# michaelklachko/NoisyNet

Hardware: NVIDIA H100
Metric: NoisyNet CIFAR-10 4-bit training images/sec (higher is better)
Workload: dtype bf16

## Files before the change

include/noisynet_b200.h:

```cpp
#ifndef NOISYNET_B200_H
#define NOISYNET_B200_H

#include <stdint.h>

#ifdef __cplusplus
extern "C" {
#endif

#define NN_ABI_VERSION 16


typedef struct nn_rng {
    uint64_t seed;
    uint64_t offset;
    const uint64_t* offset_dev;
} nn_rng;

const char* nn_last_error(void);
int nn_abi_version(void);
uint64_t nn_launch_count(void);
int nn_device_info(int device, int* sm_count, int* cc_major, int* cc_minor);
int nn_rng_advance(uint64_t* offset_dev, uint64_t inc, int device, void* stream);


int nn_quantize_fwd(const float* x, float* y, int64_t n, int bits, double min_value,
                    double max_value, float stochastic, const float* u_inject, nn_rng rng,
                    int device, void* stream);
int nn_quantize_bwd(const float* x, const float* gy, float* gx, int64_t n, double min_value,
                    double max_value, int device, void* stream);

int64_t nn_range_scratch_bytes(void);
int nn_range_select(const float* x, int64_t n, int64_t k_rank, double pctl_percent, int mode, double min_value, float* out4,
// ... 63 lines not shown
    int64_t workspace_bytes;
    const void* x_packed;
    const void* w_packed;
    int32_t w_packed_layout;
    float* pooled_out;
    uint8_t* argmax_out;
    float* bn_mean;
    float* bn_invstd;
    float* bn_running_mean;
    float* bn_running_var;
    float bn_eps, bn_momentum;
    int32_t bn_eval_mode;
    void* bn_scratch;
    float* zero_out;
} nn_conv_fwd_args;
int64_t nn_conv_bn_scratch_bytes(int Cout);
int nn_conv_linear_bn_fusable(const nn_conv_geom* g, int32_t noise_mode, int32_t precision, int device);

#define NN_PACK_TILED 0
#define NN_PACK_SHIFT 1
#define NN_PACK_TMA 2
int nn_conv_pack_layout(const nn_conv_geom* g, int32_t noise_mode, int32_t precision);
int nn_conv_dgrad_pack_layout(const nn_conv_geom* g, int32_t precision);
int nn_debug_tma_enable(int enable);
int nn_conv_pool_fusable(const nn_conv_geom* g, int32_t noise_mode, int32_t precision);
int nn_debug_shift_enable(int enable);

int64_t nn_conv_workspace_bytes(const nn_conv_geom* g, int32_t precision);
int nn_conv_supported(const nn_conv_geom* g, int32_t precision, int32_t which);
int nn_debug_error_flag(int device, int reset);
float nn_debug_main_kernel_ms(int enable);
int nn_debug_cta_timeline(long long* host_out, int max_ctas);
int nn_noisy_conv_fwd(const nn_conv_fwd_args* a, int device, void* stream);

typedef struct nn_conv_dgrad_args {
    nn_conv_geom g;
    const float* gy;
    const float* w_eff;
    float* gx;
    const float* x_pre; double x_lo, x_hi;
    int32_t precision;
    float w_code_scale;
    void* workspace; int64_t workspace_bytes;
    const void* gy_packed;
    const void* w_packed;
    int32_t w_packed_layout;
// ... 126 lines not shown
```

noisynet_b200/_lib.py:

```python
import ctypes as C
import os

_HERE = os.path.dirname(os.path.abspath(__file__))
LIB_PATH = os.environ.get("NN_LIB_PATH") or os.path.join(_HERE, "lib", "libnoisynet_b200.so")
ABI_VERSION = 16

NOISE_NONE, NOISE_MERGED, NOISE_EXTERNAL = 0, 1, 2
PREC_FP32, PREC_TF32, PREC_BF16 = 0, 1, 2
PACK_TILED, PACK_SHIFT, PACK_TMA = 0, 1, 2

c_f32p = C.c_void_p


class Rng(C.Structure):
    _fields_ = [("seed", C.c_uint64), ("offset", C.c_uint64), ("offset_dev", C.c_void_p)]


class ConvGeom(C.Structure):
    _fields_ = [("B", C.c_int32), ("Cin", C.c_int32), ("H", C.c_int32), ("W", C.c_int32),
                ("Cout", C.c_int32), ("KH", C.c_int32), ("KW", C.c_int32),
                ("stride", C.c_int32), ("pad", C.c_int32)]


class ConvFwdArgs(C.Structure):
    _fields_ = [("g", ConvGeom),
                ("x", C.c_void_p), ("w_eff", C.c_void_p), ("w_raw", C.c_void_p), ("bias", C.c_void_p),
                ("y", C.c_void_p), ("y_noisy", C.c_void_p),
                ("noise_mode", C.c_int32), ("current", C.c_float),
                ("scale_dev", C.c_void_p), ("z_inject", C.c_void_p), ("z_export", C.c_void_p),
                ("sigma_export", C.c_void_p),
                ("rng", Rng),
                ("stats", C.c_void_p),
# ... 109 lines not shown
                                  C.c_void_p, C.c_float, C.c_float, C.c_void_p, C.c_void_p, C.c_void_p, C.c_void_p,
                                  C.c_int, C.c_void_p, C.c_void_p, C.c_int, C.c_void_p]),
    "nn_allreduce_ctl_bytes": (C.c_int64, []),
    "nn_allreduce_start": (C.c_int, [C.POINTER(C.c_void_p), C.c_void_p, C.c_int, C.c_int, C.c_int, C.c_int64, C.c_int64, C.c_int,
                                     C.c_int, C.c_void_p]),
    "nn_allreduce_wait": (C.c_int, [C.c_void_p, C.c_int, C.c_int, C.c_int, C.c_void_p]),
    "nn_head_eval": (C.c_int, [C.c_void_p, C.c_int, C.c_int, C.c_void_p, C.c_void_p, C.c_void_p, C.c_void_p, C.c_float, C.c_void_p,
                               C.c_int, C.c_void_p]),
    "nn_tensor_stats": (C.c_int, [C.c_void_p, C.c_int64, C.c_void_p, C.c_int, C.c_void_p]),
    "nn_clamp_absmax": (C.c_int, [C.c_void_p, C.c_int64, C.c_float, C.c_void_p, C.c_int, C.c_void_p]),
    "nn_noise_epilogue": (C.c_int, [C.c_void_p, C.c_void_p, C.c_void_p, C.c_int64, C.c_int64, C.c_void_p,
                                    C.c_float, C.c_void_p, C.c_void_p, C.c_void_p, Rng, C.c_int, C.c_void_p]),
    "nn_alt_noise": (C.c_int, [C.c_void_p, C.c_void_p, C.c_int64, C.c_int, C.c_float, C.c_void_p,
                               C.c_void_p, Rng, C.c_int, C.c_void_p]),
    "nn_conv_workspace_bytes": (C.c_int64, [C.POINTER(ConvGeom), C.c_int32]),
    "nn_conv_supported": (C.c_int, [C.POINTER(ConvGeom), C.c_int32, C.c_int32]),
    "nn_debug_error_flag": (C.c_int, [C.c_int, C.c_int]),
    "nn_debug_main_kernel_ms": (C.c_float, [C.c_int]),
    "nn_debug_cta_timeline": (C.c_int, [C.c_void_p, C.c_int]),
    "nn_conv_pack_layout": (C.c_int, [C.POINTER(ConvGeom), C.c_int32, C.c_int32]),
    "nn_debug_shift_enable": (C.c_int, [C.c_int]),
    "nn_debug_tma_enable": (C.c_int, [C.c_int]),
    "nn_conv_dgrad_pack_layout": (C.c_int, [C.POINTER(ConvGeom), C.c_int32]),
    "nn_conv_pool_fusable": (C.c_int, [C.POINTER(ConvGeom), C.c_int32, C.c_int32]),
    "nn_classifier_tail": (C.c_int, [C.POINTER(TailArgs), C.c_int, C.c_void_p]),
    "nn_conv_wgrad_pack_layout": (C.c_int, [C.POINTER(ConvGeom), C.c_int32, C.c_int]),
    "nn_conv_gy_planes_bytes": (C.c_int64, [C.POINTER(ConvGeom)]),
    "nn_noisy_conv_fwd": (C.c_int, [C.POINTER(ConvFwdArgs), C.c_int, C.c_void_p]),
    "nn_noisy_conv_dgrad": (C.c_int, [C.POINTER(ConvDgradArgs), C.c_int, C.c_void_p]),
    "nn_conv_wgrad_workspace_bytes": (C.c_int64, [C.POINTER(ConvGeom), C.c_int32, C.c_int]),
    "nn_noisy_conv_wgrad": (C.c_int, [C.POINTER(ConvWgradArgs), C.c_int, C.c_void_p]),
}

_lib = None


class NoisyNetLibraryError(RuntimeError):
    pass


def load():
    global _lib
    if _lib is not None:
        return _lib
    if not os.path.isfile(LIB_PATH):
        raise NoisyNetLibraryError(
# ... 19 lines not shown
```

noisynet_b200/csrc/nn_conv_tma.cu:

```cuda
#include "nn_conv_tma.h"

#include <cuda.h>

#include "nn_wgmma.cuh"

namespace {

constexpr int TC_MAX_STAGES = 8;

struct TmaConvP {
    CUtensorMap map64, map_tail;
    CUtensorMap mapb64, mapb_tail;
    int M, OH, OW, Cout, stride, pad, KW, taps;
    int n_c64, tail_w, nc, gpt, n_groups;
    int n_mma, n_half, n_tiles;
    int stages, a_stage, b_stage, n_prod, tap_bytes;
    float y_scale, s_scale;
    float *y, *y_noisy;
    float current;
    const float* scale_dev;
    const float* z_inject;
    nn_rng rng;
    int* err_flag;
};
// ... 621 lines not shown
    p.taps = w.taps;
    p.partial_tail = reinterpret_cast<float*>(reinterpret_cast<uint8_t*>(c.partial) + w.main_bytes);
    p.OH = c.OH; p.OW = c.OW; p.stride = c.stride; p.pad = c.pad; p.KW = c.KW; p.n_c64 = w.n_c64; p.n_atoms = w.n_atoms;
    p.Mpix = c.B * c.OH * c.OW; p.Cout = c.Cout; p.num_kb = w.num_kb; p.kb_per_split = w.kb_per_split; p.stages = w.stages;
    p.cols_pad = w.cols_pad; p.partial = c.partial; p.err_flag = c.err_flag;
    typedef void (*WgradKernel)(const WgTmaP);
    const int tw = w.tail_w ? (w.taps * 8 + 15) & ~15 : 0;
    const WgradKernel tail = tw == 16 ? k_wgrad_tma<true, 16> : tw == 32 ? k_wgrad_tma<true, 32> : tw == 80 ? k_wgrad_tma<true, 80>
                           : tw == 128 ? k_wgrad_tma<true, 128> : tw == 208 ? k_wgrad_tma<true, 208> : nullptr;
    if (w.tail_w && !tail) return nn_fail("nn_conv_tma: no remainder weight-gradient kernel for%s %lld taps", "", (long long)w.taps);
    NN_ONCE_PER_DEVICE({
        NN_CUDA_OK(cudaFuncSetAttribute(k_wgrad_tma<false, 0>, cudaFuncAttributeMaxDynamicSharedMemorySize, 227 * 1024));
        for (WgradKernel k : {k_wgrad_tma<true, 16>, k_wgrad_tma<true, 32>, k_wgrad_tma<true, 80>, k_wgrad_tma<true, 128>, k_wgrad_tma<true, 208>})
            NN_CUDA_OK(cudaFuncSetAttribute(k, cudaFuncAttributeMaxDynamicSharedMemorySize, 227 * 1024));
    });
    k_wgrad_tma<false, 0><<<dim3(w.tiles_k, w.m_tiles_n, w.splits), WT_THREADS, w.smem_bytes, st>>>(p);
    NN_LAUNCH_OK();
    if (w.tail_w) {
        tail<<<dim3(1, w.m_tiles_n, w.splits), WT_THREADS, w.smem_bytes, st>>>(p);
        NN_LAUNCH_OK();
    }
    return 0;
}
```

noisynet_b200/csrc/nn_conv_tma.h:

```cpp
#pragma once
#include "nn_common.cuh"

struct TmaPlan {
    int Cp, taps, n_c64, tail_w, wt, nc, gpt, n_groups;
    int n_t, n_tiles, n_mma, n_half, main_col, sig_col;
    int stages, a_stage, b_stage, n_prod, threads;
    int tap_bytes;
    size_t smem_bytes, wp_bytes;
};

bool nn_tma_make_plan(int Cin_k, int KH, int KW, int stride, int pad, int n_out, bool has_sigma, int OH, int OW, TmaPlan* out);

struct TmaConvCall {
    TmaPlan pl;
    int B, H, W;
    int OH, OW, KH, KW, stride, pad;
    int Cout;
    const void* xp;
    const void* wp;
    float y_scale, s_scale;
    float* y;
    float* y_noisy;
    int noise_mode;
    float current;
// ... 1 lines not shown
    const float* z_inject;
    nn_rng rng;
    int* err_flag;
    void *ev0, *ev1;
};
int nn_tma_conv_launch(const TmaConvCall& c, int device, cudaStream_t st);

struct TmaWgradPlan {
    int Cp, Coutp, taps, n_c64, tail_w;
    int n_atoms, tiles_k, cols_pad, m_tiles_n, num_kb, kb_per_split, splits, stages;
    size_t smem_bytes, main_bytes, partial_bytes;
};
bool nn_tma_wgrad_plan(int Cin, int KH, int KW, int stride, int pad, int Cout, int64_t Mpix, int device, TmaWgradPlan* out);
struct TmaWgradCall {
    TmaWgradPlan pl;
    int B, H, W, OH, OW, KH, KW, stride, pad, Cout;
    const void* xp;
    const void* gyp;
    float* partial;
    int* err_flag;
};
int nn_tma_wgrad_launch(const TmaWgradCall& c, int device, cudaStream_t st);

int nn_tma_encode_rows(void* map_out, const void* ptr, uint64_t rows, uint64_t cols, uint64_t pitch_bytes);
```

noisynet_b200/csrc/nn_conv_umma.cu:

```cuda
#include <cuda_bf16.h>
#include <stdio.h>
#include <stdlib.h>

#include "nn_common.cuh"
#include "nn_wgmma.cuh"
#include "nn_conv_tma.h"

namespace {

constexpr int UM_BLOCK_M = 128;
constexpr int UM_BLOCK_K = 64;
constexpr int UM_THREADS = 384;
constexpr int UM_ACC_CH = 4;
constexpr int UM_A_STAGE = UM_BLOCK_M * 128;
constexpr int UM_MAX_NT = 120;

struct UmmaP {
    int B, H, W, Cp;
    int KH, KW, stride, pad, OH, OW;
    int M, Cout, n_t, n_mma, num_kb, stages, acc_cols;
    int main_col, sig_col, wsum_col;
    int ring_bytes;
    const __nv_bfloat16* xp;
    const __nv_bfloat16* wp;
// ... 892 lines not shown
            if (c < C) {
                f = __ldg(x + ((int64_t)b * C + c) * HW + p);
                if (code_scale > 0.f) f = rintf(__fdiv_rn(f, code_scale));
            }
            v[j] = __float2bfloat16_rn(f);
        }
        *reinterpret_cast<uint4*>(xp + (pixel * Cp + chunk * 8)) = *reinterpret_cast<const uint4*>(v);
    }
}

struct PackWP {
    const float *w_eff, *w_raw;
    __nv_bfloat16* wp;
    int Cout, Cin, KHW, Cp, n_t, n_mma, num_kb, n_tiles;
    int main_col, sig_col, wsum_col, noise_mode, mode;
    int layout;
    float w_code_scale;
    int q_bits;
    float q_hi, q_scale, q_max, q_stoch;
    const float* u_inject;
    nn_rng rng;
    const int8_t* codes;
    int t_nc64, t_tail, t_nc, t_wt, t_nhalf, t_tapbytes;
};

__device__ __forceinline__ float pack_main_value(const PackWP& p, const NnRng& rs, int64_t idx) {
    if (p.codes) return (float)p.codes[idx];
    if (p.q_bits > 0) {
        const float w = __ldg(p.w_raw + idx);
        float u = 0.f;
        if (p.q_stoch > 0.f) {
            if (p.u_inject) u = __ldg(p.u_inject + idx);
            else {
                const uint4 r = nn_philox(rs, (uint64_t)(idx >> 2));
                const uint32_t rr[4] = {r.x, r.y, r.z, r.w};
                u = nn_usym(rr[idx & 3], p.q_stoch);
            }
        }
        float t = __fadd_rn(__fdiv_rn(__fadd_rn(w, p.q_hi), p.q_scale), u);
        t = rintf(fminf(fmaxf(t, 0.f), p.q_max));
        return 2.f * t - p.q_max;
    }
    float f = __ldg(p.w_eff + idx);
    if (p.w_code_scale > 0.f) f = rintf(__fdiv_rn(f, p.w_code_scale));
    return f;
}

__device__ __forceinline__ void pack_w_job(const PackWP& p, int64_t start, int64_t stride) {
    const NnRng rs = nn_rng_load(p.rng);
    const bool shift = p.layout == 1, tma = p.layout == 2;
    const int64_t total = shift ? (int64_t)p.num_kb * p.n_mma
                          : tma ? (int64_t)p.n_tiles * p.n_mma * p.KHW * (p.t_wt >> 3)
                                : (int64_t)p.n_tiles * p.num_kb * p.n_mma * 8;
    for (int64_t i = start; i < total; i += stride) {
        int j, r, kb, tile, kbase;
        int tap_t = 0, c_first_t = 0;
        int64_t off_t = 0;
        if (tma) {
            const int cpt = p.t_wt >> 3;
            tap_t = (int)(i % p.KHW);
            const int qc = (int)((i / p.KHW) % cpt);
            const int R = (int)(i / ((int64_t)p.KHW * cpt));
            tile = R / p.n_mma; r = R - tile * p.n_mma;
            c_first_t = qc * 8;
            int ci = c_first_t >> 6;
            if (ci > p.t_nc64) ci = p.t_nc64;
            const int w = ci < p.t_nc64 ? 64 : p.t_tail;
            j = (c_first_t - 64 * ci) >> 3;
            const int gi = ci >> 1, slot = ci & 1;
            const int wa = (2 * gi < p.t_nc64) ? 64 : p.t_tail;
            const int wb = (2 * gi + 1 < p.t_nc) ? ((2 * gi + 1 < p.t_nc64) ? 64 : p.t_tail) : 0;
            const int rank = r / p.t_nhalf, rr = r - rank * p.t_nhalf;
            const int swz = w == 64 ? (rr & 7) : (w == 32 ? ((rr >> 1) & 3) : ((rr >> 2) & 1));
// ... 881 lines not shown
    if (p.pooled) {
        if (mode == 0) NN_SHIFT_LAUNCH(0, 16, true); else if (mode == 1) NN_SHIFT_LAUNCH(1, 16, true); else NN_SHIFT_LAUNCH(2, 16, true);
    } else {
        if (mode == 0) NN_SHIFT_LAUNCH(0, 16, false); else if (mode == 1) NN_SHIFT_LAUNCH(1, 16, false); else NN_SHIFT_LAUNCH(2, 16, false);
    }
#undef NN_SHIFT_LAUNCH
    if (g_time_main) cudaEventRecord(g_ev1, st);
    NN_LAUNCH_OK();
    return 0;
}

extern "C" int nn_conv_pack_layout(const nn_conv_geom* g, int32_t noise_mode, int32_t precision) {
    if (!g || precision != NN_PREC_BF16) return NN_PACK_TILED;
    if (make_shift_plan(*g, noise_mode != NN_NOISE_NONE, nullptr)) return NN_PACK_SHIFT;
    int OH, OW;
    nn_out_hw(*g, OH, OW);
    return nn_tma_make_plan(g->Cin, g->KH, g->KW, g->stride, g->pad, g->Cout, noise_mode != NN_NOISE_NONE, OH, OW, nullptr) ? NN_PACK_TMA
                                                                                                                          : NN_PACK_TILED;
}
extern "C" int nn_conv_dgrad_pack_layout(const nn_conv_geom* g, int32_t precision) {
    if (!g || precision != NN_PREC_BF16 || g->stride != 1) return NN_PACK_TILED;
    return nn_tma_make_plan(g->Cout, g->KH, g->KW, 1, g->KH - 1 - g->pad, g->Cin, false, g->H, g->W, nullptr) ? NN_PACK_TMA : NN_PACK_TILED;
}
extern "C" int nn_conv_pool_fusable(const nn_conv_geom* g, int32_t noise_mode, int32_t precision) {
    if (!g || precision != NN_PREC_BF16) return 0;
    if (!make_shift_plan(*g, noise_mode != NN_NOISE_NONE, nullptr)) return 0;
    int OH, OW;
    nn_out_hw(*g, OH, OW);
    const int ngrp = (g->Cout + 3) / 4;
    return g->W % 8 == 0 && g->H % 16 == 0 && OH % 2 == 0 && OW % 2 == 0 && ngrp / 4 <= SH_POOL_IT - 1 && ngrp % 4 <= 1;
}
extern "C" int nn_conv_linear_bn_fusable(const nn_conv_geom* g, int32_t noise_mode, int32_t precision, int device) {
    if (!g || precision != NN_PREC_BF16) return 0;
    int OH, OW;
    nn_out_hw(*g, OH, OW);
    const int M = g->B * OH * OW;
    if (OH * OW != 1 || M % 256 || M > 4096) return 0;
    const Plan pl = make_plan(g->Cin, g->KH * g->KW, g->Cout, true, noise_mode != NN_NOISE_NONE, false, (int64_t)g->B * g->H * g->W, (M + 127) / 128);
    const int ctas = ((M + UM_BLOCK_M - 1) / UM_BLOCK_M) * pl.n_tiles;
    return ctas * 2 <= nn_num_sms(device) && pl.num_kb >= 8 && pl.num_kb / 2 >= 4;
}
extern "C" int64_t nn_conv_bn_scratch_bytes(int Cout) { return 16 + (int64_t)256 * Cout * 2 * sizeof(double); }
extern "C" int nn_debug_shift_enable(int enable) {
    const int prev = g_shift_enable;
    if (enable >= 0) g_shift_enable = enable;
    return prev;
// ... 172 lines not shown
    return make_plan(jb.Cout, jb.KHW, jb.Cin, true, false, false, 0, (jb.m_rows + 127) / 128);
}

static void shift_plan_for_job(const nn_wprep_job& jb, ShiftPlan* sp) {
    const bool noisy = jb.noise_mode != NN_NOISE_NONE;
    sp->n_t = pad_to(jb.Cout, 8); sp->main_col = 0; sp->sig_col = noisy ? sp->n_t : -1;
    sp->n_mma = pad_to(noisy ? 2 * sp->n_t : sp->n_t, 16);
    sp->n_pairs = (jb.KHW + 1) / 2; sp->n_chunks = 2 * sp->n_pairs;
    sp->b_bytes = sp->n_chunks * sp->n_mma * 16; sp->wp_bytes = (size_t)sp->b_bytes;
}

static bool tma_plan_for_job(const nn_wprep_job& jb, TmaPlan* tp) {
    int k = 1;
    while (k * k < jb.KHW) ++k;
    if (k * k != jb.KHW) return false;
    if (jb.mode == 0) return nn_tma_make_plan(jb.Cin, k, k, 1, 0, jb.Cout, jb.noise_mode != NN_NOISE_NONE, 2, 2, tp);
    return nn_tma_make_plan(jb.Cout, k, k, 1, 0, jb.Cin, false, 2, 2, tp);
}

extern "C" int64_t nn_weight_pack_bytes(const nn_wprep_job* jb) {
    if (!jb) return 0;
    if (jb->layout == NN_PACK_TMA) { TmaPlan tp; return tma_plan_for_job(*jb, &tp) ? (int64_t)align_up(tp.wp_bytes, 1024) : 0; }
    if (jb->layout == NN_PACK_SHIFT) { ShiftPlan sp; shift_plan_for_job(*jb, &sp); return (int64_t)align_up(sp.wp_bytes, 1024); }
    return (int64_t)align_up(plan_for_job(*jb).wp_bytes, 1024);
}

extern "C" int nn_prepare_weights(const nn_wprep_job* jobs, int count, int device, void* stream) {
    if (count <= 0) return 0;
    if (count > UM_MAX_PACK_JOBS) return nn_fail("nn_prepare_weights: too many jobs%s (%lld)", "", count);
    NN_SET_DEVICE(device);
    PackJobs pj;
    memset(&pj, 0, sizeof(pj));
    int64_t max_total = 0;
    for (int i = 0; i < count; ++i) {
        const nn_wprep_job& jb = jobs[i];
        if (!jb.w_raw || !jb.packed_out) return nn_fail("nn_prepare_weights: null pointer%s", "");
        if (jb.q_bits > 0 && !(jb.q_hi > 0)) return nn_fail("nn_prepare_weights: symmetric range needs q_hi > 0%s", "");
        Plan pl = plan_for_job(jb);
        TmaPlan tp;
        if (jb.layout == NN_PACK_TMA) {
            if (jb.want_wsum || !tma_plan_for_job(jb, &tp))
                return nn_fail("nn_prepare_weights: NN_PACK_TMA is not served for this job%s (see nn_conv_pack_layout)", "");
        } else if (jb.layout == NN_PACK_SHIFT) {
            if (jb.mode != 0 || jb.Cin > 8 || jb.want_wsum)
                return nn_fail("nn_prepare_weights: NN_PACK_SHIFT needs a forward job with Cin <= 8 and no colsum row%s", "");
            ShiftPlan sp;
            shift_plan_for_job(jb, &sp);
            pl.Cp = 8; pl.n_t = sp.n_t; pl.n_mma = sp.n_mma; pl.num_kb = sp.n_chunks; pl.n_tiles = 1;
            pl.main_col = sp.main_col; pl.sig_col = sp.sig_col; pl.wsum_col = -1;
        }
        PackWP& pw = pj.j[i];
        pw.w_eff = jb.w_raw; pw.w_raw = jb.w_raw; pw.wp = (__nv_bfloat16*)jb.packed_out;
        pw.Cout = jb.Cout; pw.Cin = jb.Cin; pw.KHW = jb.KHW; pw.Cp = pl.Cp; pw.n_t = pl.n_t; pw.n_mma = pl.n_mma;
        pw.num_kb = pl.num_kb; pw.n_tiles = pl.n_tiles; pw.main_col = pl.main_col; pw.sig_col = pl.sig_col;
        pw.wsum_col = pl.wsum_col; pw.noise_mode = jb.noise_mode; pw.mode = jb.mode; pw.w_code_scale = 0.f;
        pw.layout = jb.layout;
        pw.q_bits = jb.q_bits;
        if (jb.q_bits > 0) {
            const double qmax = (double)((1u << jb.q_bits) - 1u);
            double sc = 2.0 * jb.q_hi / qmax;
            if (sc < 1e-6) sc = 1e-6;
            pw.q_hi = (float)jb.q_hi; pw.q_scale = (float)sc; pw.q_max = (float)qmax; pw.q_stoch = jb.stochastic;
            pw.u_inject = jb.u_inject; pw.rng = jb.rng;
        }
        int64_t total = jb.layout == NN_PACK_SHIFT ? (int64_t)pl.num_kb * pl.n_mma
                                                   : (int64_t)pl.n_tiles * pl.num_kb * pl.n_mma * 8;
        if (jb.layout == NN_PACK_TMA) { fill_pack_tma(pw, tp); total = pack_tma_chunks(tp); }
        if (total > max_total) max_total = total;
    }
    {
        CodeJobs cj;
        memset(&cj, 0, sizeof(cj));
        int nc = 0;
        int64_t max_groups = 0;
        for (int i = 0; i < count; ++i) {
            const nn_wprep_job& jb = jobs[i];
            if (!jb.codes || jb.q_bits <= 0) continue;
            if (jb.q_bits > 7) return nn_fail("nn_prepare_weights: the code scratch serves q_bits <= 7%s", "");
            pj.j[i].codes = (const int8_t*)jb.codes;
            bool seen = false;
            for (int k = 0; k < nc; ++k) seen = seen || cj.j[k].codes == (int8_t*)jb.codes;
            if (seen) continue;
            CodeJob& c = cj.j[nc++];
            c.w = jb.w_raw; c.codes = (int8_t*)jb.codes; c.n = (int64_t)jb.Cout * jb.Cin * jb.KHW;
            c.q_hi = pj.j[i].q_hi; c.q_scale = pj.j[i].q_scale; c.q_max = pj.j[i].q_max; c.q_stoch = pj.j[i].q_stoch;
            c.u_inject = jb.u_inject; c.rng = jb.rng;
            if ((c.n + 3) / 4 > max_groups) max_groups = (c.n + 3) / 4;
        }
        if (nc > 0) {
            int gx = (int)((max_groups + 255) / 256);
            if (gx > 4 * nn_num_sms(device)) gx = 4 * nn_num_sms(device);
            k_quant_codes<<<dim3(gx, nc), 256, 0, (cudaStream_t)stream>>>(cj);
            NN_LAUNCH_OK();
        }
    }
    int gx = (int)((max_total + 255) / 256);
    if (gx > 4 * nn_num_sms(device)) gx = 4 * nn_num_sms(device);
    dim3 grid(gx, count);
    k_pack_w_batch<<<grid, 256, 0, (cudaStream_t)stream>>>(pj);
    NN_LAUNCH_OK();
    return 0;
}

int nn_umma_conv_dgrad(const nn_conv_dgrad_args* a, int device, cudaStream_t st) {
    if (a->precision != NN_PREC_BF16)
        return nn_fail("nn_noisy_conv_dgrad: tensor-core path implements NN_PREC_BF16 only%s", "");
    const nn_conv_geom& g = a->g;
    int OH, OW;
    nn_out_hw(g, OH, OW);
    {
        TmaPlan tp;
        const bool can = !a->x_pre && g.stride == 1 &&
                         nn_tma_make_plan(g.Cout, g.KH, g.KW, 1, g.KH - 1 - g.pad, g.Cin, false, g.H, g.W, &tp);
        const int layout = a->w_packed ? a->w_packed_layout : (can ? NN_PACK_TMA : NN_PACK_TILED);
        if (layout == NN_PACK_TMA) {
            if (!can) return nn_fail("nn_noisy_conv_dgrad: w_packed_layout = NN_PACK_TMA is not served for this call%s", "");
            const size_t xp_bytes = (size_t)g.B * OH * OW * tp.Cp * 2;
            const size_t need = (a->gy_packed ? 0 : align_up(xp_bytes, 1024)) + (a->w_packed ? 0 : align_up(tp.wp_bytes, 1024)) + 1024;
            if ((!a->gy_packed || !a->w_packed) && (!a->workspace || (size_t)a->workspace_bytes < need))
                return nn_fail("nn_noisy_conv_dgrad: workspace too small%s (need %lld bytes)", "", (long long)need);
            uint8_t* ws = (uint8_t*)align_up((size_t)a->workspace, 1024);
            const void* xp = a->gy_packed;
            const void* wp = a->w_packed;
            if (!xp) {
                const int64_t total = (int64_t)g.B * OH * OW * (tp.Cp / 8);
                int grid = (int)((total + 255) / 256);
                if (grid > 16 * nn_num_sms(device)) grid = 16 * nn_num_sms(device);
                k_pack_act<<<grid, 256, 0, st>>>(a->gy, (__nv_bfloat16*)ws, g.B, g.Cout, OH * OW, tp.Cp, 0.f);
                NN_LAUNCH_OK();
                xp = ws;
                ws += align_up(xp_bytes, 1024);
            }
// ... 371 lines not shown
```

noisynet_b200/engine.py:

```python
import ctypes as C
import os

import torch

from . import _lib, ops
from ._lib import (NOISE_EXTERNAL, NOISE_MERGED, PACK_SHIFT, PREC_BF16, ConvDgradArgs, ConvFwdArgs, ConvGeom, ConvWgradArgs,
                   Rng, StageArgs, StageBwdArgs, TailArgs, WPrepJob)
from .hardware_model import _f32


def _p(t):
    return None if t is None else t.data_ptr()


class _Layer:
    pass


class NoisyNetEngine:
    def __init__(self, model, batch, opt=None, reducer=None):
        a = model.args
        self.q_w = [int(a.q_w1), int(a.q_w2), int(a.q_w3), int(a.q_w4)]
        self.q_a = [int(a.q_a1), int(a.q_a2), int(a.q_a3), int(a.q_a4)]
        if any(getattr(a, k, 0) > 0 for k in ("n_w1", "n_w2", "n_w3", "n_w4")) and min(self.q_w) == 0:
            raise NotImplementedError("NoisyNetEngine: multiplicative weight noise (--n_w) is served by the module path")
        if max(self.q_w) > 7:
            raise ValueError("NoisyNetEngine: weight codes are int8 (q_w <= 7)")
        if a.use_bias:
            raise NotImplementedError("NoisyNetEngine: bias is served by the module path (net.NoisyNet(fused=True), or the "
# ... 45 lines not shown
        modes = [NOISE_MERGED if a.merged_dac else NOISE_EXTERNAL, NOISE_EXTERNAL,
                 NOISE_MERGED if a.merged_dac else NOISE_EXTERNAL, NOISE_EXTERNAL]
        self.noise_modes = [m if a.layer_currents[i] > 0 else 0 for i, m in enumerate(modes)]
        W = self._weights()
        shapes = [(C1, 3, fs * fs), (C2, C1, fs * fs), (FC, C2, P2 * P2), (10, FC, 1)]
        self.jobs = (WPrepJob * 7)()
        self.job_layer = [0, 1, 2, 3, 3, 2, 1]
        specs = [(0, shapes[0], 0, B * H1 * H1), (1, shapes[1], 0, B * H2 * H2), (2, shapes[2], 0, B), (3, shapes[3], 0, B),
                 (3, shapes[3], 1, B), (2, (FC, C2 * P2 * P2, 1), 1, B), (1, shapes[1], 1, B * P1 * P1)]
        self.geom = [ConvGeom(B, 3, 32, 32, C1, fs, fs, 1, 0), ConvGeom(B, C1, P1, P1, C2, fs, fs, 1, 0),
                     ConvGeom(B, C2, P2, P2, FC, P2, P2, 1, 0), ConvGeom(B, FC, 1, 1, 10, 1, 1, 1, 0)]
        self.geom_fc1_lin = ConvGeom(B, C2 * P2 * P2, 1, 1, FC, 1, 1, 1, 0)
        self.fused_tail = B <= 2048 and self.q_w[3] > 0 and self.q_a[3] > 0 and os.environ.get("NN_ENGINE_FUSED_TAIL", "0") == "1"
        self.fuse_pool1 = bool(self.lib.nn_conv_pool_fusable(C.byref(self.geom[0]), self.noise_modes[0], PREC_BF16)) and \
            os.environ.get("NN_ENGINE_FUSE_POOL", "1") == "1"
        self.bn_scratch = torch.zeros(int(self.lib.nn_conv_bn_scratch_bytes(C1)), dtype=torch.uint8, device=dev)
        self.fuse_bn3 = bool(self.lib.nn_conv_linear_bn_fusable(C.byref(self.geom[2]), self.noise_modes[2], PREC_BF16, self.di)) and \
            os.environ.get("NN_ENGINE_FUSE_BN3", "1") == "1"
        self.bn3_scratch = torch.zeros(int(self.lib.nn_stage_scratch_bytes(FC)) + 64, dtype=torch.uint8, device=dev)
        self.gy1_layout = self.lib.nn_conv_wgrad_pack_layout(C.byref(self.geom[0]), PREC_BF16, self.di)
        if self.gy1_layout:
            nbytes = int(self.lib.nn_conv_gy_planes_bytes(C.byref(self.geom[0])))
            self.gyp1 = torch.zeros(nbytes // 16, 8, dtype=torch.bfloat16, device=dev)
        self.wpack = []
        self.wcodes = {}
        for j, (li, (co, ci, khw), mode, m_rows) in enumerate(specs):
            jb = self.jobs[j]
            jb.w_raw = W[li].data_ptr()
            jb.Cout, jb.Cin, jb.KHW, jb.mode, jb.m_rows = co, ci, khw, mode, m_rows
            jb.noise_mode = self.noise_modes[li] if mode == 0 else 0
            jb.want_wsum = 0
            if mode == 0:
                jb.layout = self.lib.nn_conv_pack_layout(C.byref(self.geom[li]), jb.noise_mode, PREC_BF16)
            else:
                jb.layout = self.lib.nn_conv_dgrad_pack_layout(C.byref(self.geom[li]), PREC_BF16) if li == 1 else 0
            jb.q_bits, jb.q_hi = self.q_w[li], 1.0
            if li not in self.wcodes:
                self.wcodes[li] = torch.zeros(W[li].numel() + 16, dtype=torch.int8, device=dev)
            jb.codes = self.wcodes[li].data_ptr() if self.q_w[li] > 0 else None
            buf = torch.zeros(int(self.lib.nn_weight_pack_bytes(C.byref(jb))) + 1024, dtype=torch.uint8, device=dev)
            jb.packed_out = (buf.data_ptr() + 1023) // 1024 * 1024
            self.wpack.append(buf)
        self.wp_fwd = [self.jobs[i].packed_out for i in range(4)]
        self.wp_dgrad = {3: self.jobs[4].packed_out, 2: self.jobs[5].packed_out, 1: self.jobs[6].packed_out}
        self.wp_dgrad_layout = {3: self.jobs[4].layout, 2: self.jobs[5].layout, 1: self.jobs[6].layout}
        need = 0
        for g in self.geom + [self.geom_fc1_lin]:
            need = max(need, self.lib.nn_conv_workspace_bytes(C.byref(g), PREC_BF16),
                       self.lib.nn_conv_wgrad_workspace_bytes(C.byref(g), PREC_BF16, self.di))
        self.ws = torch.empty(int(need) + 4096, dtype=torch.uint8, device=dev)
        self.overlap_wgrad = os.environ.get("NN_ENGINE_OVERLAP_WGRAD", "1") != "0"
        self.side = torch.cuda.Stream(device=dev) if self.overlap_wgrad else None
        self.ws_side = torch.empty(int(need) + 4096, dtype=torch.uint8, device=dev) if self.overlap_wgrad else None
        for p in model.parameters():
            if p.grad is None:
                p.grad = torch.zeros_like(p)
        self._keep_inj = []
        self.inject = None
# ... 328 lines not shown
```

Measured before the change: 471,600.

## Add scatter-style dgrad kernel for conv2 using per-image smem accumulation planes

Adds a new dgrad path for the second conv layer. Instead of a gather/implicit-GEMM over padded grad_output, each warpgroup multiplies weight tiles (taps x Cin rows) by one image's grad_output via WGMMA and scatter-adds the results into a padded fp32 input-gradient plane held in shared memory, then writes the plane out. A new weight pack layout (NN_PACK_SCATTER) and TMA-fed producer warp support this. It is enabled by default when the geometry is served. The cost is extra shared-memory read-modify-write traffic and serialized per-tile MMA waits.

```diff
diff --git a/include/noisynet_b200.h b/include/noisynet_b200.h
--- a/include/noisynet_b200.h
+++ b/include/noisynet_b200.h
@@ -7,7 +7,7 @@
 extern "C" {
 #endif
 
-#define NN_ABI_VERSION 16
+#define NN_ABI_VERSION 17
 
 
 typedef struct nn_rng {
@@ -117,6 +117,8 @@
 #define NN_PACK_TMA 2
 int nn_conv_pack_layout(const nn_conv_geom* g, int32_t noise_mode, int32_t precision);
 int nn_conv_dgrad_pack_layout(const nn_conv_geom* g, int32_t precision);
+#define NN_PACK_SCATTER 3
+int nn_conv_dgrad_scatter_served(const nn_conv_geom* g, int32_t precision);
 int nn_debug_tma_enable(int enable);
 int nn_conv_pool_fusable(const nn_conv_geom* g, int32_t noise_mode, int32_t precision);
 int nn_debug_shift_enable(int enable);
diff --git a/noisynet_b200/_lib.py b/noisynet_b200/_lib.py
--- a/noisynet_b200/_lib.py
+++ b/noisynet_b200/_lib.py
@@ -3,11 +3,11 @@
 
 _HERE = os.path.dirname(os.path.abspath(__file__))
 LIB_PATH = os.environ.get("NN_LIB_PATH") or os.path.join(_HERE, "lib", "libnoisynet_b200.so")
-ABI_VERSION = 16
+ABI_VERSION = 17
 
 NOISE_NONE, NOISE_MERGED, NOISE_EXTERNAL = 0, 1, 2
 PREC_FP32, PREC_TF32, PREC_BF16 = 0, 1, 2
-PACK_TILED, PACK_SHIFT, PACK_TMA = 0, 1, 2
+PACK_TILED, PACK_SHIFT, PACK_TMA, PACK_SCATTER = 0, 1, 2, 3
 
 c_f32p = C.c_void_p
 
@@ -163,6 +163,7 @@
     "nn_debug_shift_enable": (C.c_int, [C.c_int]),
     "nn_debug_tma_enable": (C.c_int, [C.c_int]),
     "nn_conv_dgrad_pack_layout": (C.c_int, [C.POINTER(ConvGeom), C.c_int32]),
+    "nn_conv_dgrad_scatter_served": (C.c_int, [C.POINTER(ConvGeom), C.c_int32]),
     "nn_conv_pool_fusable": (C.c_int, [C.POINTER(ConvGeom), C.c_int32, C.c_int32]),
     "nn_classifier_tail": (C.c_int, [C.POINTER(TailArgs), C.c_int, C.c_void_p]),
     "nn_conv_wgrad_pack_layout": (C.c_int, [C.POINTER(ConvGeom), C.c_int32, C.c_int]),
diff --git a/noisynet_b200/csrc/nn_conv_tma.cu b/noisynet_b200/csrc/nn_conv_tma.cu
--- a/noisynet_b200/csrc/nn_conv_tma.cu
+++ b/noisynet_b200/csrc/nn_conv_tma.cu
@@ -667,3 +667,245 @@
     }
     return 0;
 }
+
+namespace {
+
+constexpr int SD_MAX_STAGES = 4;
+constexpr int SD_THREADS = 9 * 32;
+
+struct ScatterDgradP {
+    CUtensorMap map_gy;
+    CUtensorMap map_w;
+    int B, n_items, OHW, OW, PW, Cin, taps, tap_rows, KW, n_mtiles, kc, stages, PS, HW, W, pad;
+    uint32_t b_bytes, a_bytes;
+    float scale;
+    float* gx;
+    int* err_flag;
+};
+
+__device__ __forceinline__ int sd_swz(int c) { return ((c & 6) << 2) | (c & 1); }
+
+template <int N, int KC>
+__device__ __forceinline__ void scatter_tile_mma(float* acc, uint64_t ad, uint64_t bd) {
+    wg_fence();
+#pragma unroll
+    for (int k = 0; k < 4; ++k) wgmma_c<N, 0, 0>(acc, ad + 2 * k, bd + 2 * k, 1);
+#pragma unroll
+    for (int k = 0; k < (KC == 2 ? 4 : 0); ++k) wgmma_c<N, 0, 0>(acc, ad + (8192 >> 4) + 2 * k, bd + ((N * 128) >> 4) + 2 * k, 1);
+    wg_commit();
+    wg_wait_all();
+}
+
+template <int N>
+__global__ void __launch_bounds__(SD_THREADS, 1)
+k_dgrad_scatter(const __grid_constant__ ScatterDgradP p) {
+    extern __shared__ uint8_t smem_raw[];
+    const uint32_t base = (smem_u32(smem_raw) + 1023u) & ~1023u;
+    const int S = p.stages;
+    const uint32_t ring = base + 2u * p.b_bytes;
+    const uint32_t plane_base = ring + (uint32_t)S * p.a_bytes;
+    const int plane_floats = p.Cin * p.PS;
+    const uint32_t bar_base = plane_base + 8u * (uint32_t)plane_floats;
+    const uint32_t full_bar = bar_base, empty_bar = bar_base + 8u * SD_MAX_STAGES;
+    const uint32_t b_full = bar_base + 16u * SD_MAX_STAGES, b_empty = b_full + 16u;
+    const int tid = threadIdx.x, lane = tid & 31;
+    const int warp = __shfl_sync(0xffffffffu, tid >> 5, 0);
+    const int T = p.n_mtiles;
+
+    if (tid == 0) {
+        for (int s = 0; s < S; ++s) { mbar_init(full_bar + 8 * s, 1); mbar_init(empty_bar + 8 * s, 2); }
+        for (int w = 0; w < 2; ++w) { mbar_init(b_full + 8 * w, 1); mbar_init(b_empty + 8 * w, 1); }
+        fence_mbar_init();
+        tma_prefetch_desc(&p.map_gy);
+        tma_prefetch_desc(&p.map_w);
+    }
+    __syncthreads();
+
+    int fail = 0;
+    if (warp == 8) {
+        int s = 0;
+        uint32_t eph = 1u, bph = 1u;
+        for (int item = blockIdx.x; item < p.n_items && !fail; item += gridDim.x) {
+            for (int w = 0; w < 2; ++w) {
+                const int img = 2 * item + w;
+                if (img >= p.B) break;
+                if (!mbar_wait_backoff(b_empty + 8 * w, bph)) { fail = 601; break; }
+                if (elect_one_sync()) {
+                    const uint32_t dst = base + (uint32_t)w * p.b_bytes;
+                    mbar_arrive_expect_tx(b_full + 8 * w, p.b_bytes);
+                    for (int c = 0; c < p.kc; ++c) tma_tile_2d(dst + (uint32_t)(c * N * 128), &p.map_gy, b_full + 8 * w, 64 * c, img * p.OHW);
+                }
+                __syncwarp();
+            }
+            bph ^= 1u;
+            for (int t = 0; t < T && !fail; ++t) {
+                if (!mbar_wait_backoff(empty_bar + 8 * s, eph)) { fail = 602; break; }
+                if (elect_one_sync()) {
+                    mbar_arrive_expect_tx(full_bar + 8 * s, p.a_bytes);
+                    tma_tile_2d(ring + (uint32_t)s * p.a_bytes, &p.map_w, full_bar + 8 * s, 0, t * 64 * p.kc);
+                }
+                __syncwarp();
+                if (++s == S) { s = 0; eph ^= 1u; }
+            }
+        }
+    } else {
+        const int wg = warp >> 2, wq = warp & 3, q = lane & 3, wt = tid & 127;
+        const uint32_t bar_wg = 1u + (uint32_t)wg;
+        const bool releaser = wq == 0;
+        float* const pl = reinterpret_cast<float*>(smem_raw + (plane_base - smem_u32(smem_raw))) + wg * plane_floats;
+        {
+            float4* z4 = reinterpret_cast<float4*>(pl);
+            for (int i = wt; i < plane_floats / 4; i += 128) z4[i] = make_float4(0.f, 0.f, 0.f, 0.f);
+        }
+        uint32_t coff[N / 8];
+#pragma unroll
+        for (int i = 0; i < N / 8; ++i) {
+            coff[i] = 0u;
+#pragma unroll
+            for (int j = 0; j < 2; ++j) {
+                const int n = 8 * i + 2 * q + j, oh = n / p.OW;
+                coff[i] |= (uint32_t)(n < p.OHW ? oh * p.PW + (n - oh * p.OW) : 0xFFFF) << (16 * j);
+            }
+        }
+        const uint64_t bd = gmma_desc_kmajor(base + (uint32_t)wg * p.b_bytes, 128u);
+        int s = 0;
+        uint32_t fph = 0u, bph = 0u;
+        float acc[N / 2];
+        for (int item = blockIdx.x; item < p.n_items && !fail; item += gridDim.x) {
+            const int img = 2 * item + wg;
+            const bool has = img < p.B;
+            if (has && !mbar_wait(b_full + 8 * wg, bph)) { fail = 603; break; }
+            bph ^= 1u;
+            for (int t = 0; t < T; ++t) {
+                if (!mbar_wait(full_bar + 8 * s, fph)) { fail = 604; break; }
+                if (has) {
+                    int roff[2];
+                    bool ok[2];
+#pragma unroll
+                    for (int h = 0; h < 2; ++h) {
+                        const int R = 64 * t + 16 * wq + (lane >> 2) + 8 * h, tq = R / p.tap_rows, ci = R - tq * p.tap_rows;
+                        const int tap = p.taps - 1 - tq, kh = tap / p.KW;
+                        ok[h] = tq < p.taps && ci < p.Cin;
+                        roff[h] = ci * p.PS + sd_swz(ci) + kh * p.PW + (tap - kh * p.KW);
+                    }
+                    named_bar_sync(bar_wg, 128);
+#pragma unroll
+                    for (int i = 0; i < N / 8; ++i)
+#pragma unroll
+                        for (int h = 0; h < 2; ++h)
+#pragma unroll
+                            for (int j = 0; j < 2; ++j) {
+                                const uint32_t c = (coff[i] >> (16 * j)) & 0xFFFFu;
+                                acc[4 * i + 2 * h + j] = ok[h] && c != 0xFFFFu ? pl[roff[h] + (int)c] : 0.f;
+                            }
+                    const uint64_t ad = gmma_desc_kmajor(ring + (uint32_t)s * p.a_bytes, 128u);
+                    if (p.kc == 2) scatter_tile_mma<N, 2>(acc, ad, bd);
+                    else scatter_tile_mma<N, 1>(acc, ad, bd);
+                    wg_fence_regs<N / 2>(acc);
+                    asm volatile("" : "+r"(roff[0]), "+r"(roff[1]));
+#pragma unroll
+                    for (int i = 0; i < N / 8; ++i)
+#pragma unroll
+                        for (int h = 0; h < 2; ++h)
+#pragma unroll
+                            for (int j = 0; j < 2; ++j) {
+                                const uint32_t c = (coff[i] >> (16 * j)) & 0xFFFFu;
+                                if (ok[h] && c != 0xFFFFu) pl[roff[h] + (int)c] = acc[4 * i + 2 * h + j];
+                            }
+                }
+                if (releaser && elect_one_sync()) {
+                    mbar_arrive(empty_bar + 8 * s);
+                    if (has && t == T - 1) mbar_arrive(b_empty + 8 * wg);
+                }
+                __syncwarp();
+                if (++s == S) { s = 0; fph ^= 1u; }
+            }
+            if (fail || !has) break;
+            named_bar_sync(bar_wg, 128);
+            for (int ci = wq; ci < p.Cin; ci += 4) {
+                const float* src = pl + ci * p.PS + sd_swz(ci);
+                float* out = p.gx + ((size_t)img * p.Cin + ci) * p.HW;
+                for (int o = lane; o < p.HW; o += 32) {
+                    const int y = o / p.W, x = o - y * p.W;
+                    out[o] = src[(y + p.pad) * p.PW + x + p.pad] * p.scale;
+                }
+            }
+            named_bar_sync(bar_wg, 128);
+            float4* z4 = reinterpret_cast<float4*>(pl);
+            for (int i = wt; i < plane_floats / 4; i += 128) z4[i] = make_float4(0.f, 0.f, 0.f, 0.f);
+        }
+    }
+    if (fail) nn_pipeline_abort(p.err_flag, fail);
+}
+
+}
+
+void nn_scatter_dgrad_image(int Cin, int Cout, int taps, int* tap_rows, int* n_mtiles, int* kc) {
+    *tap_rows = Cin > 64 ? Cin : 64;
+    *n_mtiles = (taps * *tap_rows + 63) / 64;
+    *kc = (tc_pad_to(Cout, 8) + 63) / 64;
+}
+
+bool nn_scatter_dgrad_plan(int Cin, int Cout, int KH, int KW, int stride, int pad, int H, int W, ScatterDgradPlan* out) {
+    if (KH != KW || stride != 1 || pad < 0 || Cin < 1 || Cout < 1 || Cout > 128) return false;
+    ScatterDgradPlan sp;
+    memset(&sp, 0, sizeof(sp));
+    sp.OH = H + 2 * pad - KH + 1;
+    sp.OW = W + 2 * pad - KW + 1;
+    if (sp.OH < 1 || sp.OW < 1 || pad > KH - 1) return false;
+    sp.N = tc_pad_to(sp.OH * sp.OW, 8);
+    if (sp.N != 64 && sp.N != 104) return false;
+    nn_scatter_dgrad_image(Cin, Cout, KH * KW, &sp.tap_rows, &sp.n_mtiles, &sp.kc);
+    sp.PH = sp.OH + KH - 1;
+    sp.PW = sp.OW + KW - 1;
+    sp.PS = tc_pad_to(sp.PH * sp.PW + 25, 32);
+    sp.b_bytes = (size_t)sp.kc * sp.N * 128;
+    sp.a_bytes = (size_t)sp.kc * 8192;
+    const size_t plane_bytes = (size_t)2 * Cin * sp.PS * 4;
+    const long long avail = 227 * 1024 - 1024 - 128 - (long long)plane_bytes - 2 * (long long)sp.b_bytes;
+    sp.stages = avail > 0 ? (int)(avail / (long long)sp.a_bytes) : 0;
+    if (sp.stages > SD_MAX_STAGES) sp.stages = SD_MAX_STAGES;
+    if (sp.stages < 2) return false;
+    sp.smem_bytes = 1024 + 2 * sp.b_bytes + (size_t)sp.stages * sp.a_bytes + plane_bytes + 128;
+    sp.wp_bytes = (size_t)sp.n_mtiles * sp.a_bytes;
+    if (out) *out = sp;
+    return true;
+}
+
+int nn_scatter_dgrad_launch(const ScatterDgradCall& c, int device, cudaStream_t st) {
+    const ScatterDgradPlan& sp = c.pl;
+    ScatterDgradP p;
+    memset(&p, 0, sizeof(p));
+    {
+        EncodeTiledFn enc = get_encode_tiled();
+        if (!enc) return nn_fail("nn_conv_tma: cuTensorMapEncodeTiled is not available%s", "");
+        const cuuint64_t coutp = (cuuint64_t)tc_pad_to(c.Cout, 8);
+        cuuint64_t dims[2] = {coutp, (cuuint64_t)c.B * sp.OH * sp.OW};
+        cuuint64_t strides[1] = {coutp * 2};
+        cuuint32_t box[2] = {64, (cuuint32_t)sp.N};
+        cuuint32_t estr[2] = {1, 1};
+        const CUresult r = enc(&p.map_gy, CU_TENSOR_MAP_DATA_TYPE_BFLOAT16, 2, const_cast<void*>(c.gyp), dims, strides, box, estr,
+                               CU_TENSOR_MAP_INTERLEAVE_NONE, CU_TENSOR_MAP_SWIZZLE_128B, CU_TENSOR_MAP_L2_PROMOTION_L2_128B,
+                               CU_TENSOR_MAP_FLOAT_OOB_FILL_NONE);
+        if (r != CUDA_SUCCESS) return nn_fail("nn_conv_tma: cuTensorMapEncodeTiled (scatter dgrad grad_output) failed%s (CUresult %lld)", "",
+                                              (long long)r);
+    }
+    if (((uintptr_t)c.wp & 15) != 0) return nn_fail("nn_conv_tma: the weight image must be 16-byte aligned%s", "");
+    if (int e = encode_weight_map(&p.map_w, c.wp, sp.wp_bytes, 64, 64 * sp.kc)) return e;
+    p.B = c.B; p.n_items = (c.B + 1) / 2; p.OHW = sp.OH * sp.OW; p.OW = sp.OW; p.PW = sp.PW;
+    p.Cin = c.Cin; p.taps = c.KH * c.KW; p.tap_rows = sp.tap_rows; p.KW = c.KW; p.n_mtiles = sp.n_mtiles; p.kc = sp.kc;
+    p.stages = sp.stages; p.PS = sp.PS; p.HW = c.H * c.W; p.W = c.W; p.pad = c.pad;
+    p.b_bytes = (uint32_t)sp.b_bytes; p.a_bytes = (uint32_t)sp.a_bytes;
+    p.scale = c.scale; p.gx = c.gx; p.err_flag = c.err_flag;
+    typedef void (*ScatterKernel)(const ScatterDgradP);
+    const ScatterKernel kern = sp.N == 104 ? k_dgrad_scatter<104> : k_dgrad_scatter<64>;
+    NN_ONCE_PER_DEVICE({
+        for (ScatterKernel k : {k_dgrad_scatter<64>, k_dgrad_scatter<104>})
+            NN_CUDA_OK(cudaFuncSetAttribute(k, cudaFuncAttributeMaxDynamicSharedMemorySize, 227 * 1024));
+    });
+    int grid = nn_num_sms(device);
+    if (grid > p.n_items) grid = p.n_items;
+    kern<<<grid, SD_THREADS, sp.smem_bytes, st>>>(p);
+    NN_LAUNCH_OK();
+    return 0;
+}
diff --git a/noisynet_b200/csrc/nn_conv_tma.h b/noisynet_b200/csrc/nn_conv_tma.h
--- a/noisynet_b200/csrc/nn_conv_tma.h
+++ b/noisynet_b200/csrc/nn_conv_tma.h
@@ -47,4 +47,23 @@
 };
 int nn_tma_wgrad_launch(const TmaWgradCall& c, int device, cudaStream_t st);
 
+void nn_scatter_dgrad_image(int Cin, int Cout, int taps, int* tap_rows, int* n_mtiles, int* kc);
+struct ScatterDgradPlan {
+    int OH, OW, N;
+    int tap_rows, n_mtiles, kc, PH, PW, PS;
+    int stages;
+    size_t b_bytes, a_bytes, smem_bytes, wp_bytes;
+};
+bool nn_scatter_dgrad_plan(int Cin, int Cout, int KH, int KW, int stride, int pad, int H, int W, ScatterDgradPlan* out);
+struct ScatterDgradCall {
+    ScatterDgradPlan pl;
+    int B, Cin, H, W, Cout, KH, KW, pad;
+    const void* gyp;
+    const void* wp;
+    float scale;
+    float* gx;
+    int* err_flag;
+};
+int nn_scatter_dgrad_launch(const ScatterDgradCall& c, int device, cudaStream_t st);
+
 int nn_tma_encode_rows(void* map_out, const void* ptr, uint64_t rows, uint64_t cols, uint64_t pitch_bytes);
diff --git a/noisynet_b200/csrc/nn_conv_umma.cu b/noisynet_b200/csrc/nn_conv_umma.cu
--- a/noisynet_b200/csrc/nn_conv_umma.cu
+++ b/noisynet_b200/csrc/nn_conv_umma.cu
@@ -938,6 +938,7 @@
     nn_rng rng;
     const int8_t* codes;
     int t_nc64, t_tail, t_nc, t_wt, t_nhalf, t_tapbytes;
+    int s_tap_rows, s_kc, s_mtiles;
 };
 
 __device__ __forceinline__ float pack_main_value(const PackWP& p, const NnRng& rs, int64_t idx) {
@@ -965,6 +966,24 @@
 __device__ __forceinline__ void pack_w_job(const PackWP& p, int64_t start, int64_t stride) {
     const NnRng rs = nn_rng_load(p.rng);
     const bool shift = p.layout == 1, tma = p.layout == 2;
+    if (p.layout == NN_PACK_SCATTER) {
+        const int64_t total = (int64_t)p.s_mtiles * p.s_kc * 64 * 8;
+        for (int64_t i = start; i < total; i += stride) {
+            const int j = (int)(i & 7), r = (int)((i >> 3) & 63);
+            const int64_t tk = i >> 9;
+            const int chunk = (int)(tk % p.s_kc), R = (int)(tk / p.s_kc) * 64 + r;
+            const int tq = R / p.s_tap_rows, ci = R - tq * p.s_tap_rows, tap = p.KHW - 1 - tq;
+            __align__(16) __nv_bfloat16 v[8];
+#pragma unroll
+            for (int e = 0; e < 8; ++e) {
+                const int co = chunk * 64 + 8 * j + e;
+                const bool live = tq < p.KHW && ci < p.Cin && co < p.Cout;
+                v[e] = __float2bfloat16_rn(live ? pack_main_value(p, rs, ((int64_t)co * p.Cin + ci) * p.KHW + tap) : 0.f);
+            }
+            *reinterpret_cast<uint4*>(p.wp + ((tk * 64 + r) * 64 + ((j ^ (r & 7)) << 3))) = *reinterpret_cast<const uint4*>(v);
+        }
+        return;
+    }
     const int64_t total = shift ? (int64_t)p.num_kb * p.n_mma
                           : tma ? (int64_t)p.n_tiles * p.n_mma * p.KHW * (p.t_wt >> 3)
                                 : (int64_t)p.n_tiles * p.num_kb * p.n_mma * 8;
@@ -1892,6 +1911,10 @@
     if (!g || precision != NN_PREC_BF16 || g->stride != 1) return NN_PACK_TILED;
     return nn_tma_make_plan(g->Cout, g->KH, g->KW, 1, g->KH - 1 - g->pad, g->Cin, false, g->H, g->W, nullptr) ? NN_PACK_TMA : NN_PACK_TILED;
 }
+extern "C" int nn_conv_dgrad_scatter_served(const nn_conv_geom* g, int32_t precision) {
+    if (!g || precision != NN_PREC_BF16) return 0;
+    return nn_scatter_dgrad_plan(g->Cin, g->Cout, g->KH, g->KW, g->stride, g->pad, g->H, g->W, nullptr) ? 1 : 0;
+}
 extern "C" int nn_conv_pool_fusable(const nn_conv_geom* g, int32_t noise_mode, int32_t precision) {
     if (!g || precision != NN_PREC_BF16) return 0;
     if (!make_shift_plan(*g, noise_mode != NN_NOISE_NONE, nullptr)) return 0;
@@ -2110,6 +2133,12 @@
     if (!jb) return 0;
     if (jb->layout == NN_PACK_TMA) { TmaPlan tp; return tma_plan_for_job(*jb, &tp) ? (int64_t)align_up(tp.wp_bytes, 1024) : 0; }
     if (jb->layout == NN_PACK_SHIFT) { ShiftPlan sp; shift_plan_for_job(*jb, &sp); return (int64_t)align_up(sp.wp_bytes, 1024); }
+    if (jb->layout == NN_PACK_SCATTER) {
+        if (jb->mode != 1 || jb->Cout > 128) return 0;
+        int tap_rows, n_mtiles, kc;
+        nn_scatter_dgrad_image(jb->Cin, jb->Cout, jb->KHW, &tap_rows, &n_mtiles, &kc);
+        return (int64_t)n_mtiles * kc * 8192;
+    }
     return (int64_t)align_up(plan_for_job(*jb).wp_bytes, 1024);
 }
 
@@ -2129,6 +2158,9 @@
         if (jb.layout == NN_PACK_TMA) {
             if (jb.want_wsum || !tma_plan_for_job(jb, &tp))
                 return nn_fail("nn_prepare_weights: NN_PACK_TMA is not served for this job%s (see nn_conv_pack_layout)", "");
+        } else if (jb.layout == NN_PACK_SCATTER) {
+            if (jb.mode != 1 || jb.Cout > 128 || jb.want_wsum)
+                return nn_fail("nn_prepare_weights: NN_PACK_SCATTER needs a dgrad job with Cout <= 128%s", "");
         } else if (jb.layout == NN_PACK_SHIFT) {
             if (jb.mode != 0 || jb.Cin > 8 || jb.want_wsum)
                 return nn_fail("nn_prepare_weights: NN_PACK_SHIFT needs a forward job with Cin <= 8 and no colsum row%s", "");
@@ -2154,6 +2186,10 @@
         int64_t total = jb.layout == NN_PACK_SHIFT ? (int64_t)pl.num_kb * pl.n_mma
                                                    : (int64_t)pl.n_tiles * pl.num_kb * pl.n_mma * 8;
         if (jb.layout == NN_PACK_TMA) { fill_pack_tma(pw, tp); total = pack_tma_chunks(tp); }
+        if (jb.layout == NN_PACK_SCATTER) {
+            nn_scatter_dgrad_image(jb.Cin, jb.Cout, jb.KHW, &pw.s_tap_rows, &pw.s_mtiles, &pw.s_kc);
+            total = (int64_t)pw.s_mtiles * pw.s_kc * 64 * 8;
+        }
         if (total > max_total) max_total = total;
     }
     {
@@ -2196,6 +2232,20 @@
     const nn_conv_geom& g = a->g;
     int OH, OW;
     nn_out_hw(g, OH, OW);
+    if (a->w_packed && a->w_packed_layout == NN_PACK_SCATTER) {
+        ScatterDgradPlan sp;
+        if (a->x_pre || !a->gy_packed || !nn_scatter_dgrad_plan(g.Cin, g.Cout, g.KH, g.KW, g.stride, g.pad, g.H, g.W, &sp))
+            return nn_fail("nn_noisy_conv_dgrad: w_packed_layout = NN_PACK_SCATTER is not served for this call%s "
+                           "(see nn_conv_dgrad_scatter_served; gy_packed required, no x_pre)", "");
+        ScatterDgradCall c;
+        memset(&c, 0, sizeof(c));
+        c.pl = sp;
+        c.B = g.B; c.Cin = g.Cin; c.H = g.H; c.W = g.W; c.Cout = g.Cout; c.KH = g.KH; c.KW = g.KW; c.pad = g.pad;
+        c.gyp = a->gy_packed; c.wp = a->w_packed; c.gx = a->gx;
+        c.scale = a->w_code_scale > 0.f ? a->w_code_scale : 1.f;
+        c.err_flag = nn_umma_err_flag(device);
+        return nn_scatter_dgrad_launch(c, device, st);
+    }
     {
         TmaPlan tp;
         const bool can = !a->x_pre && g.stride == 1 &&
diff --git a/noisynet_b200/engine.py b/noisynet_b200/engine.py
--- a/noisynet_b200/engine.py
+++ b/noisynet_b200/engine.py
@@ -4,7 +4,7 @@
 import torch
 
 from . import _lib, ops
-from ._lib import (NOISE_EXTERNAL, NOISE_MERGED, PACK_SHIFT, PREC_BF16, ConvDgradArgs, ConvFwdArgs, ConvGeom, ConvWgradArgs,
+from ._lib import (NOISE_EXTERNAL, NOISE_MERGED, PACK_SCATTER, PACK_SHIFT, PREC_BF16, ConvDgradArgs, ConvFwdArgs, ConvGeom, ConvWgradArgs,
                    Rng, StageArgs, StageBwdArgs, TailArgs, WPrepJob)
 from .hardware_model import _f32
 
@@ -96,6 +96,8 @@
         if self.gy1_layout:
             nbytes = int(self.lib.nn_conv_gy_planes_bytes(C.byref(self.geom[0])))
             self.gyp1 = torch.zeros(nbytes // 16, 8, dtype=torch.bfloat16, device=dev)
+        self.scatter_dgrad = bool(self.lib.nn_conv_dgrad_scatter_served(C.byref(self.geom[1]), PREC_BF16)) and \
+            os.environ.get("NN_ENGINE_SCATTER_DGRAD", "1") == "1"
         self.wpack = []
         self.wcodes = {}
         for j, (li, (co, ci, khw), mode, m_rows) in enumerate(specs):
@@ -106,8 +108,10 @@
             jb.want_wsum = 0
             if mode == 0:
                 jb.layout = self.lib.nn_conv_pack_layout(C.byref(self.geom[li]), jb.noise_mode, PREC_BF16)
+            elif li == 1:
+                jb.layout = PACK_SCATTER if self.scatter_dgrad else self.lib.nn_conv_dgrad_pack_layout(C.byref(self.geom[li]), PREC_BF16)
             else:
-                jb.layout = self.lib.nn_conv_dgrad_pack_layout(C.byref(self.geom[li]), PREC_BF16) if li == 1 else 0
+                jb.layout = 0
             jb.q_bits, jb.q_hi = self.q_w[li], 1.0
             if li not in self.wcodes:
                 self.wcodes[li] = torch.zeros(W[li].numel() + 16, dtype=torch.int8, device=dev)
```

New measurement: 507,000 (median of 6 runs). 1.08x the previous value.
